# isabella232/handel

Measured on AMD Instinct MI355X. Metric: BN254 aggregate-sig verifications/sec (batch 4096), higher is better.
Workload: dtype u32 (26-bit-limb Fp, 64-bit accumulators)

## Files before the change

### handel_amd/build.py

```python

from __future__ import annotations

import os
import subprocess
import sys
from concurrent.futures import ThreadPoolExecutor

HERE = os.path.dirname(os.path.abspath(__file__))
CSRC = os.path.join(HERE, "csrc")
OUT_DIR = os.path.join(HERE, "_build")
LIB = os.path.join(OUT_DIR, "libhandel_gpu.so")
DIAG_LIB = os.path.join(OUT_DIR, "libhandel_gpu_diag.so")
SOURCES = ["bn256_verify.hip", "bn256_pair.hip", "bn256_kernels.hip", "bn256_gt.hip", "bn256_sig12.hip", "bn256_sigw2.hip", "hg_api.cpp", "hg_aggregate.cpp", "hg_intake.cpp",
           "hg_batcher.cpp", "hg_packets.hip", "hg_service.cpp", "hg_stores.hip", "hg_merge.hip"]
HEADERS = ["bn256_fp.h", "bn256_curve.h", "bn256_team.h", "bn256_kernels.h", "bn256_constants.h",
           "bn256_g2team.h", "bn256_g2sched.h", "bn256_pairing.h", "bn256_xprog.h", "bn256_xtab.h", "bn256_redq.h", "bn256_inv.h", "bn256_agg.h", "bn256_gt.h", "bn256_decode.h", "hg_packets.h", "hg_stores.h", "hg_shm.h", "hg_codes.h", "hg_dev.h", "hg_ctx.h", "hg_sha256.h", "bn256_sigfe.h", "bn256_sigteam.h", "bn256_sigsplit.h", "bn256_sigform.h"]
ARCH = os.environ.get("HG_OFFLOAD_ARCH", "gfx950")
HIPCC = os.environ.get("HIPCC", "/opt/rocm/bin/hipcc")
CFLAGS = ["-O3", "-fPIC", "-std=c++17", f"--offload-arch={ARCH}", "-Wno-unused-result"]


def _inputs():
    files = [os.path.join(CSRC, f) for f in SOURCES + HEADERS]
    files.append(os.path.join(HERE, "..", "include", "handel_gpu.h"))
    files.append(os.path.abspath(__file__))
    return files


def up_to_date(lib: str = LIB) -> bool:
    if not os.path.exists(lib):
        return False
# ... 111 lines not shown
```

### handel_amd/csrc/bn256_sig12.hip

```cpp
#include <hip/hip_runtime.h>

#include "bn256_decode.h"
#include "bn256_g2sched.h"
#include "bn256_gt.h"
#include "bn256_sigfe.h"

namespace hg {

#ifndef HG_SIG_LINE_BLOCK
#define HG_SIG_LINE_BLOCK 256
#endif
static constexpr int kLineBlock = HG_SIG_LINE_BLOCK;

__global__ __launch_bounds__(kLineBlock) void k_sig_scalars(const uint8_t* sig_bytes, int flavor, int n, Fp* sc) {
  const int c = blockIdx.x * kLineBlock + threadIdx.x;
  if (c >= n) return;
  PointG1 sg;
  (void)decode_g1_one(sig_bytes + (size_t)c * 64, flavor, sg);
  Fp nsy, z;
  fp_zero(z);
  fp_neg(nsy, sg.y);
  const bool use = sg.inf == 0;
  fp_sel(sc[2 * c], use, sg.x, z);
  fp_sel(sc[2 * c + 1], use, nsy, z);
// ... 25 lines not shown
      const uint2 x = src[i];
      P.c.l[2 * i] = x.x;
      P.c.l[2 * i + 1] = x.y;
    }
  }
}
HG_DEV void ev_publish(const Team& T, uint32_t* F, EvPipe& P, const Fp* ev, int n, int ci, int next) {
  if (T.tl < 4) st_fp_a8(F + (R_FB_x + T.tl) * 10, P.c.l);
  team_sync();
  if (next < kNumLines) ev_fetch(T, P, ev, n, ci, next);
}

using ISqr12T = XInst<XP_SQR12_12_T, S_F, S_F>;
using ILineT = XInst<XP_LINE_FIX_12_T, S_F, S_F>;

HG_DEV void team_miller_sig12(const Team& T, uint32_t* F, const Fp* ev, int n, int ci, XStream& S, XHint after) {
  const int8_t naf[kNafLen] = HG_NAF;
  t12_set_one(T, S_F);
  if (T.tl == 0) {
    Fp zero, one;
    fp_zero(zero);
    fp_one(one);
    st_fp(F + R_ZERO * 10, zero);
    st_fp(F + R_ONE * 10, one);
  }
  team_sync();
  EvPipe P;
  fp_zero(P.c);
  ev_fetch(T, P, ev, n, ci, 0);
  int s = 0;
  for (int i = kNafLen - 1; i > 0; i--) {
    const int d = naf[i - 1];
    ev_publish(T, F, P, ev, n, ci, s + 1);
    ISqr12T::run(T, S, xh<ILineT>());
    const XHint after_digit = i > 1 ? xh<ISqr12T>() : xh<ILineT>();
    if (d != 0) {
      ILineT::run(T, S, xh<ILineT>());
      ev_publish(T, F, P, ev, n, ci, s + 2);
      ILineT::run(T, S, after_digit);
      s += 2;
    } else {
      ILineT::run(T, S, after_digit);
      s += 1;
    }
  }
  ev_publish(T, F, P, ev, n, ci, s + 1);
// ... 251 lines not shown
```

### handel_amd/csrc/bn256_xprog.h

```cpp
#pragma once
#include <utility>

#include "bn256_redq.h"
#include "bn256_team.h"

namespace hg {

struct Team;
struct XHint {
  int off, w;
};
struct XStream;
template <int NV, int NT, int NP, int NL, int W, int NP2, int NL2, int KP, int KL1, int KL2, int KS1, int KS2, int LZ,
          int EF, int FU>
HG_DEV void x_round(const Team& T, XStream& S, int off, XHint nxt);
template <int QM>
struct XQ {
  template <int NV, int NT, int NP, int NL, int W, int NP2, int NL2, int KP, int KL1, int KL2, int KS1, int KS2,
            int LZ, int EF, int FU>
  HG_DEV static void x_round(const Team& T, XStream& S, int off, XHint nxt);
};

}

#include "bn256_xtab.h"

namespace hg {

static constexpr uint32_t kP2N[10] = {HG_P2N};

struct XStream {
  uint32_t w[kXFetchWords];
  int off;
};
HG_DEV void x_fetch(const Team& T, XStream& S, XHint h) {
  const uint32_t* src = kXTab + h.off + T.tl * h.w;
// ... 48 lines not shown
  for (int l = 0; l < 10; l++) acc[l] = K >= 0 ? (uint32_t)K * kP2N[l] : 0u;
  uint32_t negk = 0;
  x_for<NT>([&](auto t) {
    const uint32_t off = x_term_off(w, base + t);
    const int32_t c = x_coef(w, base + t);
    Fp x;
    ld_fp_a8(x, x_at(T, off));
    if constexpr (K < 0) negk += c < 0 ? (uint32_t)-c : 0u;
#pragma unroll
    for (int l = 0; l < 10; l++) acc[l] += (uint32_t)c * x.l[l];
  });
#pragma unroll
  for (int l = 0; l < 10; l++) out[l] = K >= 0 ? acc[l] : acc[l] + negk * kP2N[l];
}

template <int W, int NT, int K>
HG_DEV void x_lincomb_sum(const uint32_t (&w)[W], int base, const Fp (&xs)[NT], uint32_t (&out)[10]) {
  uint32_t acc[10];
#pragma unroll
  for (int l = 0; l < 10; l++) acc[l] = K >= 0 ? (uint32_t)K * kP2N[l] : 0u;
  uint32_t negk = 0;
#pragma unroll
  for (int t = 0; t < NT; t++) {
    const int32_t c = x_coef(w, base + t);
    if constexpr (K < 0) negk += c < 0 ? (uint32_t)-c : 0u;
#pragma unroll
    for (int l = 0; l < 10; l++) acc[l] += (uint32_t)c * xs[t].l[l];
  }
#pragma unroll
  for (int l = 0; l < 10; l++) out[l] = K >= 0 ? acc[l] : acc[l] + negk * kP2N[l];
}

// ... 235 lines not shown
        const uint32_t dst = x_off(w, (P + kSplitWaves * h) * (1 + NT));
        if (dst != 0xffffu) st_fp_a8(x_at(T, dst), val[h]);
      });
    }
  };
  if constexpr (kSplitWaves == 2) {
    if (T.wave == 0) part(std::integral_constant<int, 0>{});
    else part(std::integral_constant<int, 1>{});
  } else {
    x_for<kSplitWaves>([&](auto r) {
      if (T.wave == decltype(r)::value) part(r);
    });
  }
}

template <int QM, int NV, int NT, int NP, int NL, int W, int NP2, int NL2, int KP, int KL1, int KL2, int KS1, int KS2,
          int LZ, int EF, int FU>
HG_DEV void x_round_q(const Team& T, XStream& S, int off, XHint nxt) {
  if (S.off != off) x_fetch(T, S, XHint{off, W});
  uint32_t w[W];
  x_for<W>([&](auto i) { w[i] = S.w[i]; });
  if (nxt.off >= 0) x_fetch(T, S, nxt);
  constexpr int jbase = NV * (1 + NT);
  Fp e0, e1;
  if constexpr (EF) {
    ld_fp_a8(e0, x_at(T, x_off(w, jbase)));
    ld_fp_a8(e1, x_at(T, x_off(w, jbase + 1)));
  }
  if constexpr (NV > 0) {
    if (kTeamSplit && kSplitPrepass && T.split) {
      x_prepass_split<NV, NT, W, KP>(T, w);
      team_sync(T);
    } else {
    Fp xs[NV][NT];
    x_for<NV>([&](auto v) {
      x_for<NT>([&](auto t) { ld_fp_a8(xs[v][t], x_at(T, x_term_off(w, v * (1 + NT) + 1 + t))); });
    });
    __builtin_amdgcn_sched_barrier(0);
    uint32_t val[NV][10];
    x_for<NV>([&](auto v) { x_lincomb_sum<W, NT, KP>(w, v * (1 + NT) + 1, xs[v], val[v]); });
#pragma unroll
    for (int v = 0; v < NV; v++)
#pragma unroll
      for (int l = 0; l < 10; l++) asm volatile("" : "+v"(val[v][l]));
    x_for<NV>([&](auto v) {
      const uint32_t dst = x_off(w, v * (1 + NT));
      if (dst != 0xffffu) st_fp_a8(x_at(T, dst), val[v]);
    });
    team_sync();
    }
  }
  if constexpr (kTeamSplit && NP2 == 0 && NL2 == 0) {
    if (T.split) {
      x_job_split<W, NP, NL, KL1, KS1, LZ, EF, QM>(T, w, jbase, e0, e1);
      return;
    }
  }
  Fp r;
  uint32_t dst;
  if constexpr (EF) x_job<W, NP, NL, KL1, KS1, LZ, EF, FU, QM>(T, w, jbase, r, dst, e0, e1);
  else x_job<W, NP, NL, KL1, KS1, LZ, 0, FU, QM>(T, w, jbase, r, dst);
  if constexpr (NP2 > 0 || NL2 > 0) {
// ... 3 lines not shown
    team_sync(T);
    if (!kTeamSplit || !T.split || T.wave == 0) {
      if (dst != 0xffffu) st_fp_a8(x_at(T, dst), r.l);
      if (dst2 != 0xffffu) st_fp_a8(x_at(T, dst2), r2.l);
    }
  } else {
    team_sync(T);
    if (dst != 0xffffu) st_fp_a8(x_at(T, dst), r.l);
  }
  team_sync(T);
}

template <int NV, int NT, int NP, int NL, int W, int NP2, int NL2, int KP, int KL1, int KL2, int KS1, int KS2, int LZ,
          int EF, int FU>
HG_DEV void x_round(const Team& T, XStream& S, int off, XHint nxt) {
  x_round_q<0, NV, NT, NP, NL, W, NP2, NL2, KP, KL1, KL2, KS1, KS2, LZ, EF, FU>(T, S, off, nxt);
}
template <int QM>
template <int NV, int NT, int NP, int NL, int W, int NP2, int NL2, int KP, int KL1, int KL2, int KS1, int KS2, int LZ,
          int EF, int FU>
HG_DEV void XQ<QM>::x_round(const Team& T, XStream& S, int off, XHint nxt) {
  static_assert(NL > 0 && NP2 == 0 && NL2 == 0, "one-chain rounds: one job with linear terms");
  x_round_q<QM, NV, NT, NP, NL, W, NP2, NL2, KP, KL1, KL2, KS1, KS2, LZ, EF, FU>(T, S, off, nxt);
}

template <int D, int A, int B>
using IMul12 = XInst<XP_MUL12, D, A, B>;
template <int D, int A>
using ICyc = XInst<XP_CYC_SQR_X, D, A>;
template <int D, int A>
using ICyc0 = XInst<XP_CYC_SQR, D, A>;
template <int D, int A>
using ISqr12 = XInst<XP_SQR12, D, A>;
template <int D, int A>
using ILinePk = XInst<XP_LINE_PK, D, A>;
template <int D, int A>
using ILineFix = XInst<XP_LINE_FIX, D, A>;
template <int PROG>
// ... 55 lines not shown
```

### handel_amd/csrc/bn256_xtab.h

```cpp
#pragma once
#include <stdint.h>
namespace hg {
#define HG_P2N 0x0422599cu, 0x04ac6c5du, 0x05678616u, 0x05120b5au, 0x07b96e22u, 0x0584dc20u, 0x07fb2e17u, 0x047f9aa5u, 0x078d2a8du, 0x008fb500u
enum XProg { XP_PDBL, XP_PADD_POS, XP_PADD_NEG, XP_PADD_F1, XP_PADD_F2, XP_MDBL_1, XP_MDBL_2, XP_PDBL_1, XP_PADD_POS_1, XP_MADD_POS_2, XP_PADD_POS_3, XP_PADD_NEG_1, XP_MADD_NEG_2, XP_PADD_NEG_3, XP_PADD_F1_1, XP_MADD_F1_2, XP_PADD_F1_3, XP_PADD_F2_1, XP_MADD_F2_2, XP_PADD_F2_3, XP_SQR12, XP_LINE_PK, XP_LINE_FIX, XP_CYC_SQR, XP_MUL12, XP_CYC_SQR_X, XP_FEVAL, XP_SDBL, XP_LFEV, XP_MUL12F, XP_SQR12_12, XP_LINE_FIX_12, XP_MUL12_12, XP_CYC_SQR_X_12, XP_LINE_FIX_S, XP_MUL12_S, XP_CYC_SQR_X_S, XP_FEVAL_S, XP_SDBL_S, XP_LFEV_S, XP_SQR12_12_T, XP_LINE_FIX_12_T, XP_MUL12_12_T, XP_CYC_SQR_X_12_T, XP_MDBL_1_V, XP_MDBL_2_V, XP_PDBL_1_V, XP_PADD_POS_1_V, XP_MADD_POS_2_V, XP_PADD_POS_3_V, XP_PADD_NEG_1_V, XP_MADD_NEG_2_V, XP_PADD_NEG_3_V, XP_PADD_F1_1_V, XP_MADD_F1_2_V, XP_PADD_F1_3_V, XP_PADD_F2_1_V, XP_MADD_F2_2_V, XP_PADD_F2_3_V, XP_LINE_PK_V };
__constant__ static const uint32_t kXTab[28288] = {
  0x240616d0u, 0x19509000u, 0x90002906u, 0x28ee1bd0u, 0x16d09000u, 0x16f805c8u, 0x172006b8u, 0x16801748u, 0x24fe1680u, 0x00000f00u, 0x2a1216f8u, 0x19789000u,
  0x900028fau, 0x29fa1bf8u, 0x16d09000u, 0x177006b8u, 0x16800690u, 0x16801680u, 0x2a021680u, 0x00000ff0u, 0x2a031720u, 0x19a02b03u, 0x25032403u, 0x9000ffffu,
  0x17989000u, 0x17c00618u, 0x17e80708u, 0x16801810u, 0x28fe1680u, 0x00000fa0u, 0x2aff1748u, 0x19c82b01u, 0x250124ffu, 0x9000ffffu, 0x17989000u, 0x18380708u,
  0x168006e0u, 0x16801680u, 0x2e021680u, 0x00001090u, 0x25061770u, 0x19f09000u, 0x2b092a09u, 0x9000ffffu, 0x18609000u, 0x18880668u, 0x18b00758u, 0x168018d8u,
  0x2cfe1680u, 0x00001040u, 0x26061798u, 0x1a189000u, 0x90002afau, 0x9000ffffu, 0x19009000u, 0x19280758u, 0x19500730u, 0x19780758u, 0x26020730u, 0x00000f50u,
  0x2c1217c0u, 0x1a409000u, 0x900024fau, 0x9000ffffu, 0x19a09000u, 0x19f019c8u, 0x1a181748u, 0x168006b8u, 0x25fe1680u, 0x00000f28u, 0x2c0317e8u, 0x1a682d03u,
  0x27032603u, 0x9000ffffu, 0x17709000u, 0x1a4006b8u, 0x16800690u, 0x16801680u, 0x2b021680u, 0x00001018u, 0x2cff1810u, 0x1a902d01u, 0x270126ffu, 0x9000ffffu,
  0x1a689000u, 0x1ab81a90u, 0x1ae01810u, 0x16800708u, 0x29fe1680u, 0x00000fc8u, 0x27061838u, 0x1ab89000u, 0x2d092c09u, 0x9000ffffu, 0x18389000u, 0x1b080708u,
  0x168006e0u, 0x16801680u, 0x2f021680u, 0x000010b8u, 0x28061860u, 0x1ae09000u, 0x90002cfau, 0x9000ffffu, 0x1b309000u, 0x1b801b58u, 0x1ba818d8u, 0x16800758u,
  0x2dfe1680u, 0x00001068u, 0x2e121888u, 0x1b089000u, 0x900026fau, 0x9000ffffu, 0x19289000u, 0x1bd00758u, 0x19780730u, 0x1bf80758u, 0x27020730u, 0x00000f78u,
  0x2e0318b0u, 0x1b302f03u, 0x29032803u, 0x9000ffffu, 0x16809000u, 0x16801680u, 0x16801680u, 0x16801680u, 0x90001680u, 0x0000ffffu, 0x2eff18d8u, 0x1b582f01u,
  0x290128ffu, 0x9000ffffu, 0x16809000u, 0x16801680u, 0x16801680u, 0x16801680u, 0x90001680u, 0x0000ffffu, 0x28121900u, 0x1b809000u, 0x2f092e09u, 0x9000ffffu,
  0x16809000u, 0x16801680u, 0x16801680u, 0x16801680u, 0x90001680u, 0x0000ffffu, 0x29121928u, 0x1ba89000u, 0x90002efau, 0x9000ffffu, 0x16809000u, 0x16801680u,
  0x16801680u, 0x16801680u, 0x90001680u, 0x0000ffffu, 0x0c0616d0u, 0x19509000u, 0x0f010effu, 0x020816d0u, 0x02f816f8u, 0x17481720u, 0x01e00cfeu, 0x121216f8u,
  0x19789000u, 0x900014fau, 0x17981770u, 0x02f817c0u, 0x174817e8u, 0x02080dfeu, 0x12031720u, 0x19a01303u, 0x15091409u, 0x03981810u, 0x03701838u, 0x16801680u,
  0x02300e02u, 0x12ff1748u, 0x19c81301u, 0x90000d06u, 0x03981838u, 0x18601810u, 0x16801680u, 0x02580f02u, 0x0c031770u, 0x19f00d03u, 0x90000cfau, 0x02581888u,
  0x034818b0u, 0x190018d8u, 0x028010feu, 0x0cff1798u, 0x1a180d01u, 0x90001006u, 0x19501928u, 0x03481978u, 0x190019a0u, 0x02a811feu, 0x12fa17c0u, 0x1a409000u,
  0x90001612u, 0x02f816d0u, 0x02d019c8u, 0x16801680u, 0x02d01202u, 0x120917e8u, 0x1a681309u, 0x17031603u, 0x02f819c8u, 0x02d019f0u, 0x16801680u, 0x02f81302u,
  0x10121810u, 0x1a901106u, 0x170116ffu, 0x02a81a18u, 0x03981a40u, 0x1a901a68u, 0x032014feu, 0x10fa1838u, 0x1ab81112u, 0x11031003u, 0x1ae01ab8u, 0x03981b08u,
// ... 2436 lines not shown
template <> struct XInst<XP_MUL12_S, S_B, S_A, S_B> { static constexpr int kOff = 16672, kW = 16; HG_DEV static void run(const Team& T, XStream& S, XHint h) { x_round<2, 2, 12, 0, 16, 0, 0, 4, 0, 0, 1, 0, 0, 1, 1>(T, S, 16672, h); } };
template <> struct XInst<XP_MUL12_S, S_B, S_A, S_G> { static constexpr int kOff = 16928, kW = 16; HG_DEV static void run(const Team& T, XStream& S, XHint h) { x_round<2, 2, 12, 0, 16, 0, 0, 4, 0, 0, 1, 0, 0, 1, 1>(T, S, 16928, h); } };
template <> struct XInst<XP_MUL12_S, S_B, S_C, S_G> { static constexpr int kOff = 17184, kW = 16; HG_DEV static void run(const Team& T, XStream& S, XHint h) { x_round<2, 2, 12, 0, 16, 0, 0, 4, 0, 0, 1, 0, 0, 1, 1>(T, S, 17184, h); } };
template <> struct XInst<XP_MUL12_S, S_D, S_C, S_C> { static constexpr int kOff = 17440, kW = 16; HG_DEV static void run(const Team& T, XStream& S, XHint h) { x_round<2, 2, 12, 0, 16, 0, 0, 4, 0, 0, 1, 0, 0, 1, 1>(T, S, 17440, h); } };
template <> struct XInst<XP_MUL12_S, S_D, S_D, S_B> { static constexpr int kOff = 17696, kW = 16; HG_DEV static void run(const Team& T, XStream& S, XHint h) { x_round<2, 2, 12, 0, 16, 0, 0, 4, 0, 0, 1, 0, 0, 1, 1>(T, S, 17696, h); } };
template <> struct XInst<XP_MUL12_S, S_D, S_D, S_E> { static constexpr int kOff = 17952, kW = 16; HG_DEV static void run(const Team& T, XStream& S, XHint h) { x_round<2, 2, 12, 0, 16, 0, 0, 4, 0, 0, 1, 0, 0, 1, 1>(T, S, 17952, h); } };
template <> struct XInst<XP_MUL12_S, S_D, S_D, S_G> { static constexpr int kOff = 18208, kW = 16; HG_DEV static void run(const Team& T, XStream& S, XHint h) { x_round<2, 2, 12, 0, 16, 0, 0, 4, 0, 0, 1, 0, 0, 1, 1>(T, S, 18208, h); } };
template <> struct XInst<XP_MUL12_S, S_E, S_E, S_D> { static constexpr int kOff = 18464, kW = 16; HG_DEV static void run(const Team& T, XStream& S, XHint h) { x_round<2, 2, 12, 0, 16, 0, 0, 4, 0, 0, 1, 0, 0, 1, 1>(T, S, 18464, h); } };
template <> struct XInst<XP_MUL12_S, S_E, S_E, S_G> { static constexpr int kOff = 18720, kW = 16; HG_DEV static void run(const Team& T, XStream& S, XHint h) { x_round<2, 2, 12, 0, 16, 0, 0, 4, 0, 0, 1, 0, 0, 1, 1>(T, S, 18720, h); } };
template <> struct XInst<XP_MUL12_S, S_E, S_F, S_D> { static constexpr int kOff = 18976, kW = 16; HG_DEV static void run(const Team& T, XStream& S, XHint h) { x_round<2, 2, 12, 0, 16, 0, 0, 4, 0, 0, 1, 0, 0, 1, 1>(T, S, 18976, h); } };
template <> struct XInst<XP_MUL12_S, S_F, S_B, S_A> { static constexpr int kOff = 19232, kW = 16; HG_DEV static void run(const Team& T, XStream& S, XHint h) { x_round<2, 2, 12, 0, 16, 0, 0, 4, 0, 0, 1, 0, 0, 1, 1>(T, S, 19232, h); } };
template <> struct XInst<XP_MUL12_S, S_F, S_D, S_A> { static constexpr int kOff = 19488, kW = 16; HG_DEV static void run(const Team& T, XStream& S, XHint h) { x_round<2, 2, 12, 0, 16, 0, 0, 4, 0, 0, 1, 0, 0, 1, 1>(T, S, 19488, h); } };
template <> struct XInst<XP_MUL12_S, S_F, S_F, S_A> { static constexpr int kOff = 19744, kW = 16; HG_DEV static void run(const Team& T, XStream& S, XHint h) { x_round<2, 2, 12, 0, 16, 0, 0, 4, 0, 0, 1, 0, 0, 1, 1>(T, S, 19744, h); } };
template <> struct XInst<XP_MUL12_S, S_G, S_B, S_E> { static constexpr int kOff = 20000, kW = 16; HG_DEV static void run(const Team& T, XStream& S, XHint h) { x_round<2, 2, 12, 0, 16, 0, 0, 4, 0, 0, 1, 0, 0, 1, 1>(T, S, 20000, h); } };
template <> struct XInst<XP_SDBL_S, S_F, S_F> { static constexpr int kOff = 20256, kW = 12; HG_DEV static void run(const Team& T, XStream& S, XHint h) { x_round<3, 2, 7, 0, 12, 0, 0, 8, 0, 0, 1, 0, 0, 0, 1>(T, S, 20256, h); } };
template <> struct XInst<XP_CYC_SQR_X_12_T, S_A, S_A> { static constexpr int kOff = 20448, kW = 7; HG_DEV static void run(const Team& T, XStream& S, XHint h) { XQ<13>::x_round<2, 2, 3, 1, 7, 0, 0, 4, 2, 0, 1, 0, 1, 0, 0>(T, S, 20448, h); } };
template <> struct XInst<XP_CYC_SQR_X_12_T, S_B, S_A> { static constexpr int kOff = 20560, kW = 7; HG_DEV static void run(const Team& T, XStream& S, XHint h) { XQ<13>::x_round<2, 2, 3, 1, 7, 0, 0, 4, 2, 0, 1, 0, 1, 0, 0>(T, S, 20560, h); } };
template <> struct XInst<XP_CYC_SQR_X_12_T, S_C, S_B> { static constexpr int kOff = 20672, kW = 7; HG_DEV static void run(const Team& T, XStream& S, XHint h) { XQ<13>::x_round<2, 2, 3, 1, 7, 0, 0, 4, 2, 0, 1, 0, 1, 0, 0>(T, S, 20672, h); } };
template <> struct XInst<XP_CYC_SQR_X_12_T, S_C, S_C> { static constexpr int kOff = 20784, kW = 7; HG_DEV static void run(const Team& T, XStream& S, XHint h) { XQ<13>::x_round<2, 2, 3, 1, 7, 0, 0, 4, 2, 0, 1, 0, 1, 0, 0>(T, S, 20784, h); } };
template <> struct XInst<XP_CYC_SQR_X_12_T, S_C, S_D> { static constexpr int kOff = 20896, kW = 7; HG_DEV static void run(const Team& T, XStream& S, XHint h) { XQ<13>::x_round<2, 2, 3, 1, 7, 0, 0, 4, 2, 0, 1, 0, 1, 0, 0>(T, S, 20896, h); } };
template <> struct XInst<XP_CYC_SQR_X_12_T, S_C, S_F> { static constexpr int kOff = 21008, kW = 7; HG_DEV static void run(const Team& T, XStream& S, XHint h) { XQ<13>::x_round<2, 2, 3, 1, 7, 0, 0, 4, 2, 0, 1, 0, 1, 0, 0>(T, S, 21008, h); } };
template <> struct XInst<XP_CYC_SQR_X_12_T, S_D, S_C> { static constexpr int kOff = 21120, kW = 7; HG_DEV static void run(const Team& T, XStream& S, XHint h) { XQ<13>::x_round<2, 2, 3, 1, 7, 0, 0, 4, 2, 0, 1, 0, 1, 0, 0>(T, S, 21120, h); } };
template <> struct XInst<XP_CYC_SQR_X_12_T, S_D, S_D> { static constexpr int kOff = 21232, kW = 7; HG_DEV static void run(const Team& T, XStream& S, XHint h) { XQ<13>::x_round<2, 2, 3, 1, 7, 0, 0, 4, 2, 0, 1, 0, 1, 0, 0>(T, S, 21232, h); } };
template <> struct XInst<XP_LINE_FIX_12_T, S_F, S_F> { static constexpr int kOff = 21344, kW = 7; HG_DEV static void run(const Team& T, XStream& S, XHint h) { XQ<13>::x_round<1, 2, 4, 2, 7, 0, 0, 4, 1, 0, 1, 0, 0, 1, 0>(T, S, 21344, h); } };
template <> struct XInst<XP_MUL12_12_T, S_A, S_D, S_B> { static constexpr int kOff = 21456, kW = 16; HG_DEV static void run(const Team& T, XStream& S, XHint h) { x_round<2, 2, 12, 0, 16, 0, 0, 4, 0, 0, 1, 0, 0, 1, 0>(T, S, 21456, h); } };
template <> struct XInst<XP_MUL12_12_T, S_B, S_A, S_B> { static constexpr int kOff = 21712, kW = 16; HG_DEV static void run(const Team& T, XStream& S, XHint h) { x_round<2, 2, 12, 0, 16, 0, 0, 4, 0, 0, 1, 0, 0, 1, 0>(T, S, 21712, h); } };
template <> struct XInst<XP_MUL12_12_T, S_B, S_A, S_F> { static constexpr int kOff = 21968, kW = 16; HG_DEV static void run(const Team& T, XStream& S, XHint h) { x_round<2, 2, 12, 0, 16, 0, 0, 4, 0, 0, 1, 0, 0, 1, 0>(T, S, 21968, h); } };
template <> struct XInst<XP_MUL12_12_T, S_B, S_F, S_D> { static constexpr int kOff = 22224, kW = 16; HG_DEV static void run(const Team& T, XStream& S, XHint h) { x_round<2, 2, 12, 0, 16, 0, 0, 4, 0, 0, 1, 0, 0, 1, 0>(T, S, 22224, h); } };
template <> struct XInst<XP_MUL12_12_T, S_C, S_C, S_B> { static constexpr int kOff = 22480, kW = 16; HG_DEV static void run(const Team& T, XStream& S, XHint h) { x_round<2, 2, 12, 0, 16, 0, 0, 4, 0, 0, 1, 0, 0, 1, 0>(T, S, 22480, h); } };
template <> struct XInst<XP_MUL12_12_T, S_C, S_C, S_D> { static constexpr int kOff = 22736, kW = 16; HG_DEV static void run(const Team& T, XStream& S, XHint h) { x_round<2, 2, 12, 0, 16, 0, 0, 4, 0, 0, 1, 0, 0, 1, 0>(T, S, 22736, h); } };
template <> struct XInst<XP_MUL12_12_T, S_C, S_C, S_F> { static constexpr int kOff = 22992, kW = 16; HG_DEV static void run(const Team& T, XStream& S, XHint h) { x_round<2, 2, 12, 0, 16, 0, 0, 4, 0, 0, 1, 0, 0, 1, 0>(T, S, 22992, h); } };
template <> struct XInst<XP_MUL12_12_T, S_D, S_A, S_A> { static constexpr int kOff = 23248, kW = 16; HG_DEV static void run(const Team& T, XStream& S, XHint h) { x_round<2, 2, 12, 0, 16, 0, 0, 4, 0, 0, 1, 0, 0, 1, 0>(T, S, 23248, h); } };
template <> struct XInst<XP_MUL12_12_T, S_D, S_B, S_C> { static constexpr int kOff = 23504, kW = 16; HG_DEV static void run(const Team& T, XStream& S, XHint h) { x_round<2, 2, 12, 0, 16, 0, 0, 4, 0, 0, 1, 0, 0, 1, 0>(T, S, 23504, h); } };
template <> struct XInst<XP_MUL12_12_T, S_D, S_D, S_B> { static constexpr int kOff = 23760, kW = 16; HG_DEV static void run(const Team& T, XStream& S, XHint h) { x_round<2, 2, 12, 0, 16, 0, 0, 4, 0, 0, 1, 0, 0, 1, 0>(T, S, 23760, h); } };
template <> struct XInst<XP_MUL12_12_T, S_D, S_D, S_C> { static constexpr int kOff = 24016, kW = 16; HG_DEV static void run(const Team& T, XStream& S, XHint h) { x_round<2, 2, 12, 0, 16, 0, 0, 4, 0, 0, 1, 0, 0, 1, 0>(T, S, 24016, h); } };
template <> struct XInst<XP_MUL12_12_T, S_D, S_D, S_F> { static constexpr int kOff = 24272, kW = 16; HG_DEV static void run(const Team& T, XStream& S, XHint h) { x_round<2, 2, 12, 0, 16, 0, 0, 4, 0, 0, 1, 0, 0, 1, 0>(T, S, 24272, h); } };
template <> struct XInst<XP_MUL12_12_T, S_F, S_A, S_D> { static constexpr int kOff = 24528, kW = 16; HG_DEV static void run(const Team& T, XStream& S, XHint h) { x_round<2, 2, 12, 0, 16, 0, 0, 4, 0, 0, 1, 0, 0, 1, 0>(T, S, 24528, h); } };
template <> struct XInst<XP_MUL12_12_T, S_F, S_A, S_F> { static constexpr int kOff = 24784, kW = 16; HG_DEV static void run(const Team& T, XStream& S, XHint h) { x_round<2, 2, 12, 0, 16, 0, 0, 4, 0, 0, 1, 0, 0, 1, 0>(T, S, 24784, h); } };
template <> struct XInst<XP_MUL12_12_T, S_F, S_B, S_A> { static constexpr int kOff = 25040, kW = 16; HG_DEV static void run(const Team& T, XStream& S, XHint h) { x_round<2, 2, 12, 0, 16, 0, 0, 4, 0, 0, 1, 0, 0, 1, 0>(T, S, 25040, h); } };
template <> struct XInst<XP_MUL12_12_T, S_F, S_C, S_F> { static constexpr int kOff = 25296, kW = 16; HG_DEV static void run(const Team& T, XStream& S, XHint h) { x_round<2, 2, 12, 0, 16, 0, 0, 4, 0, 0, 1, 0, 0, 1, 0>(T, S, 25296, h); } };
template <> struct XInst<XP_MUL12_12_T, S_F, S_F, S_A> { static constexpr int kOff = 25552, kW = 16; HG_DEV static void run(const Team& T, XStream& S, XHint h) { x_round<2, 2, 12, 0, 16, 0, 0, 4, 0, 0, 1, 0, 0, 1, 0>(T, S, 25552, h); } };
template <> struct XInst<XP_SQR12_12_T, S_F, S_F> { static constexpr int kOff = 25808, kW = 12; HG_DEV static void run(const Team& T, XStream& S, XHint h) { x_round<3, 2, 7, 0, 12, 0, 0, 8, 0, 0, 1, 0, 0, 0, 0>(T, S, 25808, h); } };
template <> struct XInst<XP_MDBL_1_V, S_F, S_F> { static constexpr int kOff = 26000, kW = 16; HG_DEV static void run(const Team& T, XStream& S, XHint h) { x_round<4, 2, 7, 0, 16, 2, 0, -1, -1, -1, 1, 0, 0, 0, 0>(T, S, 26000, h); } };
template <> struct XInst<XP_MDBL_2_V, S_F, S_F> { static constexpr int kOff = 26256, kW = 14; HG_DEV static void run(const Team& T, XStream& S, XHint h) { x_round<2, 4, 4, 2, 14, 2, 2, -1, -1, -1, 1, 0, 0, 0, 0>(T, S, 26256, h); } };
template <> struct XInst<XP_PDBL_1_V> { static constexpr int kOff = 26480, kW = 4; HG_DEV static void run(const Team& T, XStream& S, XHint h) { x_round<1, 2, 2, 0, 4, 0, 0, -1, -1, -1, 0, 0, 0, 0, 0>(T, S, 26480, h); } };
template <> struct XInst<XP_LINE_PK_V, S_F, S_F> { static constexpr int kOff = 26544, kW = 8; HG_DEV static void run(const Team& T, XStream& S, XHint h) { x_round<1, 2, 6, 0, 8, 0, 0, 4, 0, 0, 1, 0, 0, 1, 0>(T, S, 26544, h); } };
template <> struct XInst<XP_PADD_POS_1_V> { static constexpr int kOff = 26672, kW = 5; HG_DEV static void run(const Team& T, XStream& S, XHint h) { x_round<1, 2, 2, 1, 5, 0, 0, 1, 0, 0, 0, 0, 0, 0, 0>(T, S, 26672, h); } };
template <> struct XInst<XP_PADD_POS_3_V> { static constexpr int kOff = 26752, kW = 10; HG_DEV static void run(const Team& T, XStream& S, XHint h) { x_round<2, 2, 6, 0, 10, 0, 0, 4, 0, 0, 1, 0, 0, 0, 0>(T, S, 26752, h); } };
template <> struct XInst<XP_PADD_NEG_1_V> { static constexpr int kOff = 26912, kW = 5; HG_DEV static void run(const Team& T, XStream& S, XHint h) { x_round<1, 2, 2, 1, 5, 0, 0, 1, 0, 0, 0, 0, 0, 0, 0>(T, S, 26912, h); } };
template <> struct XInst<XP_PADD_NEG_3_V> { static constexpr int kOff = 26992, kW = 10; HG_DEV static void run(const Team& T, XStream& S, XHint h) { x_round<2, 2, 6, 0, 10, 0, 0, 4, 0, 0, 1, 0, 0, 0, 0>(T, S, 26992, h); } };
template <> struct XInst<XP_PADD_F1_1_V> { static constexpr int kOff = 27152, kW = 5; HG_DEV static void run(const Team& T, XStream& S, XHint h) { x_round<1, 2, 2, 1, 5, 0, 0, 1, 0, 0, 0, 0, 0, 0, 0>(T, S, 27152, h); } };
template <> struct XInst<XP_PADD_F1_3_V> { static constexpr int kOff = 27232, kW = 10; HG_DEV static void run(const Team& T, XStream& S, XHint h) { x_round<2, 2, 6, 0, 10, 0, 0, 4, 0, 0, 1, 0, 0, 0, 0>(T, S, 27232, h); } };
template <> struct XInst<XP_PADD_F2_1_V> { static constexpr int kOff = 27392, kW = 5; HG_DEV static void run(const Team& T, XStream& S, XHint h) { x_round<1, 2, 2, 1, 5, 0, 0, 1, 0, 0, 0, 0, 0, 0, 0>(T, S, 27392, h); } };
template <> struct XInst<XP_PADD_F2_3_V> { static constexpr int kOff = 27472, kW = 10; HG_DEV static void run(const Team& T, XStream& S, XHint h) { x_round<2, 2, 6, 0, 10, 0, 0, 4, 0, 0, 1, 0, 0, 0, 0>(T, S, 27472, h); } };
template <> struct XInst<XP_MADD_POS_2_V, S_F, S_F> { static constexpr int kOff = 27632, kW = 10; HG_DEV static void run(const Team& T, XStream& S, XHint h) { x_round<1, 2, 4, 2, 10, 2, 0, 4, 1, 0, 1, 0, 0, 0, 0>(T, S, 27632, h); } };
template <> struct XInst<XP_MADD_NEG_2_V, S_F, S_F> { static constexpr int kOff = 27792, kW = 10; HG_DEV static void run(const Team& T, XStream& S, XHint h) { x_round<1, 2, 4, 2, 10, 2, 0, 4, 1, 0, 1, 0, 0, 0, 0>(T, S, 27792, h); } };
template <> struct XInst<XP_MADD_F1_2_V, S_F, S_F> { static constexpr int kOff = 27952, kW = 10; HG_DEV static void run(const Team& T, XStream& S, XHint h) { x_round<1, 2, 4, 2, 10, 2, 0, 4, 1, 0, 1, 0, 0, 0, 0>(T, S, 27952, h); } };
// ... 3 lines not shown
```

Baseline: 6.476 million.

## Use 64-bit mad lincomb in Fp12 rounds and peel first Miller iteration

Adds a 64-bit multiply-accumulate linear-combination path (lincomb_mad) and switches the Fp12 mul, sqr and cyclotomic-square rounds of the sig12 pipeline to it, storing results with plain word stores. It also peels the first Miller-loop step: instead of setting F to one and squaring, F is initialised directly to the first line value. This drops a redundant square and possibly a line multiply. The risks are a different instruction mix and extra register pressure from the 64-bit accumulators, and subtle correctness in the peeled initialisation.

After: 6.532 million (median of 6 runs). About the same (+0.9%).

```diff
diff --git a/handel_amd/build.py b/handel_amd/build.py
--- a/handel_amd/build.py
+++ b/handel_amd/build.py
@@ -14,7 +14,7 @@
 SOURCES = ["bn256_verify.hip", "bn256_pair.hip", "bn256_kernels.hip", "bn256_gt.hip", "bn256_sig12.hip", "bn256_sigw2.hip", "hg_api.cpp", "hg_aggregate.cpp", "hg_intake.cpp",
            "hg_batcher.cpp", "hg_packets.hip", "hg_service.cpp", "hg_stores.hip", "hg_merge.hip"]
 HEADERS = ["bn256_fp.h", "bn256_curve.h", "bn256_team.h", "bn256_kernels.h", "bn256_constants.h",
-           "bn256_g2team.h", "bn256_g2sched.h", "bn256_pairing.h", "bn256_xprog.h", "bn256_xtab.h", "bn256_redq.h", "bn256_inv.h", "bn256_agg.h", "bn256_gt.h", "bn256_decode.h", "hg_packets.h", "hg_stores.h", "hg_shm.h", "hg_codes.h", "hg_dev.h", "hg_ctx.h", "hg_sha256.h", "bn256_sigfe.h", "bn256_sigteam.h", "bn256_sigsplit.h", "bn256_sigform.h"]
+           "bn256_g2team.h", "bn256_g2sched.h", "bn256_pairing.h", "bn256_xprog.h", "bn256_xtab.h", "bn256_redq.h", "bn256_lincomb.h", "bn256_inv.h", "bn256_agg.h", "bn256_gt.h", "bn256_decode.h", "hg_packets.h", "hg_stores.h", "hg_shm.h", "hg_codes.h", "hg_dev.h", "hg_ctx.h", "hg_sha256.h", "bn256_sigfe.h", "bn256_sigteam.h", "bn256_sigsplit.h", "bn256_sigform.h"]
 ARCH = os.environ.get("HG_OFFLOAD_ARCH", "gfx950")
 HIPCC = os.environ.get("HIPCC", "/opt/rocm/bin/hipcc")
 CFLAGS = ["-O3", "-fPIC", "-std=c++17", f"--offload-arch={ARCH}", "-Wno-unused-result"]
diff --git a/handel_amd/csrc/bn256_lincomb.h b/handel_amd/csrc/bn256_lincomb.h
--- /dev/null
+++ b/handel_amd/csrc/bn256_lincomb.h
@@ -0,0 +1,39 @@
+#pragma once
+#include <stdint.h>
+
+#ifndef HG_HD
+#if defined(__HIPCC__)
+#define HG_HD __host__ __device__ __forceinline__
+#else
+#define HG_HD inline
+#endif
+#endif
+
+#if defined(__HIP_DEVICE_COMPILE__)
+#define HG_PIN64(x) asm("" : "+v"(x))
+#else
+#define HG_PIN64(x) (void)(x)
+#endif
+
+namespace hg {
+
+template <int NT, int K, class E>
+HG_HD void lincomb_mad(const int32_t (&c)[NT], const E (&xs)[NT], const uint32_t (&p2n)[10], uint32_t (&out)[10]) {
+  uint32_t negk = 0;
+  if (K < 0) {
+#pragma unroll
+    for (int t = 0; t < NT; t++) negk += c[t] < 0 ? (uint32_t)-c[t] : 0u;
+  }
+#pragma unroll
+  for (int l = 0; l < 10; l++) {
+    uint64_t acc = K >= 0 ? (uint64_t)((uint32_t)K * p2n[l]) : (uint64_t)negk * p2n[l];
+#pragma unroll
+    for (int t = 0; t < NT; t++) {
+      acc += (uint64_t)(uint32_t)c[t] * xs[t].l[l];
+      HG_PIN64(acc);
+    }
+    out[l] = (uint32_t)acc;
+  }
+}
+
+}
diff --git a/handel_amd/csrc/bn256_sig12.hip b/handel_amd/csrc/bn256_sig12.hip
--- a/handel_amd/csrc/bn256_sig12.hip
+++ b/handel_amd/csrc/bn256_sig12.hip
@@ -63,9 +63,21 @@
 using ISqr12T = XInst<XP_SQR12_12_T, S_F, S_F>;
 using ILineT = XInst<XP_LINE_FIX_12_T, S_F, S_F>;
 
+HG_DEV void sig12_set_line(const Team& T, uint32_t* F) {
+  Fp v, one;
+  fp_zero(v);
+  fp_one(one);
+  if (T.e < 4) ld_fp_a8(v, F + (R_FB_x + (T.e ^ 2)) * 10);
+  fp_sel(v, T.e == 7, one, v);
+  if (T.active) st_fp_a8(slot(T, S_F) + T.e * 10, v.l);
+  team_sync();
+}
+
 HG_DEV void team_miller_sig12(const Team& T, uint32_t* F, const Fp* ev, int n, int ci, XStream& S, XHint after) {
   const int8_t naf[kNafLen] = HG_NAF;
-  t12_set_one(T, S_F);
+  static_assert(kNafLen >= 3, "a first digit and a loop after it");
+  const bool first_adds = naf[kNafLen - 2] != 0;
+  x_fetch(T, S, first_adds ? xh<ILineT>() : xh<ISqr12T>());
   if (T.tl == 0) {
     Fp zero, one;
     fp_zero(zero);
@@ -73,12 +85,18 @@
     st_fp(F + R_ZERO * 10, zero);
     st_fp(F + R_ONE * 10, one);
   }
-  team_sync();
   EvPipe P;
   fp_zero(P.c);
   ev_fetch(T, P, ev, n, ci, 0);
-  int s = 0;
-  for (int i = kNafLen - 1; i > 0; i--) {
+  ev_publish(T, F, P, ev, n, ci, 1);
+  sig12_set_line(T, F);
+  int s = 1;
+  if (first_adds) {
+    ev_publish(T, F, P, ev, n, ci, 2);
+    ILineT::run(T, S, xh<ISqr12T>());
+    s = 2;
+  }
+  for (int i = kNafLen - 2; i > 0; i--) {
     const int d = naf[i - 1];
     ev_publish(T, F, P, ev, n, ci, s + 1);
     ISqr12T::run(T, S, xh<ILineT>());
diff --git a/handel_amd/csrc/bn256_xprog.h b/handel_amd/csrc/bn256_xprog.h
--- a/handel_amd/csrc/bn256_xprog.h
+++ b/handel_amd/csrc/bn256_xprog.h
@@ -1,6 +1,7 @@
 #pragma once
 #include <utility>
 
+#include "bn256_lincomb.h"
 #include "bn256_redq.h"
 #include "bn256_team.h"
 
@@ -20,6 +21,17 @@
             int LZ, int EF, int FU>
   HG_DEV static void x_round(const Team& T, XStream& S, int off, XHint nxt);
 };
+struct XM {
+  template <int NV, int NT, int NP, int NL, int W, int NP2, int NL2, int KP, int KL1, int KL2, int KS1, int KS2,
+            int LZ, int EF, int FU>
+  HG_DEV static void x_round(const Team& T, XStream& S, int off, XHint nxt);
+  template <int QM>
+  struct XQ {
+    template <int NV, int NT, int NP, int NL, int W, int NP2, int NL2, int KP, int KL1, int KL2, int KS1, int KS2,
+              int LZ, int EF, int FU>
+    HG_DEV static void x_round(const Team& T, XStream& S, int off, XHint nxt);
+  };
+};
 
 }
 
@@ -98,8 +110,21 @@
   for (int l = 0; l < 10; l++) out[l] = K >= 0 ? acc[l] : acc[l] + negk * kP2N[l];
 }
 
-template <int W, int NT, int K>
+HG_DEV void x_store_words(const Team& T, uint32_t byte_off, const uint32_t (&v)[10]) {
+  uint32_t* p = (uint32_t*)((uint8_t*)T.base + byte_off);
+#pragma unroll
+  for (int l = 0; l < 10; l++) p[l] = v[l];
+}
+
+template <int W, int NT, int K, int MA = 0>
 HG_DEV void x_lincomb_sum(const uint32_t (&w)[W], int base, const Fp (&xs)[NT], uint32_t (&out)[10]) {
+  if constexpr (MA) {
+    int32_t c[NT];
+#pragma unroll
+    for (int t = 0; t < NT; t++) c[t] = x_coef(w, base + t);
+    lincomb_mad<NT, K>(c, xs, kP2N, out);
+    return;
+  }
   uint32_t acc[10];
 #pragma unroll
   for (int l = 0; l < 10; l++) acc[l] = K >= 0 ? (uint32_t)K * kP2N[l] : 0u;
@@ -365,8 +390,8 @@
   }
 }
 
-template <int QM, int NV, int NT, int NP, int NL, int W, int NP2, int NL2, int KP, int KL1, int KL2, int KS1, int KS2,
-          int LZ, int EF, int FU>
+template <int QM, int MA, int NV, int NT, int NP, int NL, int W, int NP2, int NL2, int KP, int KL1, int KL2, int KS1,
+          int KS2, int LZ, int EF, int FU>
 HG_DEV void x_round_q(const Team& T, XStream& S, int off, XHint nxt) {
   if (S.off != off) x_fetch(T, S, XHint{off, W});
   uint32_t w[W];
@@ -389,14 +414,17 @@
     });
     __builtin_amdgcn_sched_barrier(0);
     uint32_t val[NV][10];
-    x_for<NV>([&](auto v) { x_lincomb_sum<W, NT, KP>(w, v * (1 + NT) + 1, xs[v], val[v]); });
+    x_for<NV>([&](auto v) { x_lincomb_sum<W, NT, KP, MA>(w, v * (1 + NT) + 1, xs[v], val[v]); });
 #pragma unroll
     for (int v = 0; v < NV; v++)
 #pragma unroll
       for (int l = 0; l < 10; l++) asm volatile("" : "+v"(val[v][l]));
     x_for<NV>([&](auto v) {
       const uint32_t dst = x_off(w, v * (1 + NT));
-      if (dst != 0xffffu) st_fp_a8(x_at(T, dst), val[v]);
+      if (dst != 0xffffu) {
+        if constexpr (MA) x_store_words(T, dst, val[v]);
+        else st_fp_a8(x_at(T, dst), val[v]);
+      }
     });
     team_sync();
     }
@@ -430,14 +458,27 @@
 template <int NV, int NT, int NP, int NL, int W, int NP2, int NL2, int KP, int KL1, int KL2, int KS1, int KS2, int LZ,
           int EF, int FU>
 HG_DEV void x_round(const Team& T, XStream& S, int off, XHint nxt) {
-  x_round_q<0, NV, NT, NP, NL, W, NP2, NL2, KP, KL1, KL2, KS1, KS2, LZ, EF, FU>(T, S, off, nxt);
+  x_round_q<0, 0, NV, NT, NP, NL, W, NP2, NL2, KP, KL1, KL2, KS1, KS2, LZ, EF, FU>(T, S, off, nxt);
 }
 template <int QM>
 template <int NV, int NT, int NP, int NL, int W, int NP2, int NL2, int KP, int KL1, int KL2, int KS1, int KS2, int LZ,
           int EF, int FU>
 HG_DEV void XQ<QM>::x_round(const Team& T, XStream& S, int off, XHint nxt) {
   static_assert(NL > 0 && NP2 == 0 && NL2 == 0, "one-chain rounds: one job with linear terms");
-  x_round_q<QM, NV, NT, NP, NL, W, NP2, NL2, KP, KL1, KL2, KS1, KS2, LZ, EF, FU>(T, S, off, nxt);
+  x_round_q<QM, 0, NV, NT, NP, NL, W, NP2, NL2, KP, KL1, KL2, KS1, KS2, LZ, EF, FU>(T, S, off, nxt);
+}
+
+template <int NV, int NT, int NP, int NL, int W, int NP2, int NL2, int KP, int KL1, int KL2, int KS1, int KS2, int LZ,
+          int EF, int FU>
+HG_DEV void XM::x_round(const Team& T, XStream& S, int off, XHint nxt) {
+  x_round_q<0, 1, NV, NT, NP, NL, W, NP2, NL2, KP, KL1, KL2, KS1, KS2, LZ, EF, FU>(T, S, off, nxt);
+}
+template <int QM>
+template <int NV, int NT, int NP, int NL, int W, int NP2, int NL2, int KP, int KL1, int KL2, int KS1, int KS2, int LZ,
+          int EF, int FU>
+HG_DEV void XM::XQ<QM>::x_round(const Team& T, XStream& S, int off, XHint nxt) {
+  static_assert(NL > 0 && NP2 == 0 && NL2 == 0, "one-chain rounds: one job with linear terms");
+  x_round_q<QM, 1, NV, NT, NP, NL, W, NP2, NL2, KP, KL1, KL2, KS1, KS2, LZ, EF, FU>(T, S, off, nxt);
 }
 
 template <int D, int A, int B>
diff --git a/handel_amd/csrc/bn256_xtab.h b/handel_amd/csrc/bn256_xtab.h
--- a/handel_amd/csrc/bn256_xtab.h
+++ b/handel_amd/csrc/bn256_xtab.h
@@ -2474,33 +2474,33 @@
 template <> struct XInst<XP_MUL12_S, S_F, S_F, S_A> { static constexpr int kOff = 19744, kW = 16; HG_DEV static void run(const Team& T, XStream& S, XHint h) { x_round<2, 2, 12, 0, 16, 0, 0, 4, 0, 0, 1, 0, 0, 1, 1>(T, S, 19744, h); } };
 template <> struct XInst<XP_MUL12_S, S_G, S_B, S_E> { static constexpr int kOff = 20000, kW = 16; HG_DEV static void run(const Team& T, XStream& S, XHint h) { x_round<2, 2, 12, 0, 16, 0, 0, 4, 0, 0, 1, 0, 0, 1, 1>(T, S, 20000, h); } };
 template <> struct XInst<XP_SDBL_S, S_F, S_F> { static constexpr int kOff = 20256, kW = 12; HG_DEV static void run(const Team& T, XStream& S, XHint h) { x_round<3, 2, 7, 0, 12, 0, 0, 8, 0, 0, 1, 0, 0, 0, 1>(T, S, 20256, h); } };
-template <> struct XInst<XP_CYC_SQR_X_12_T, S_A, S_A> { static constexpr int kOff = 20448, kW = 7; HG_DEV static void run(const Team& T, XStream& S, XHint h) { XQ<13>::x_round<2, 2, 3, 1, 7, 0, 0, 4, 2, 0, 1, 0, 1, 0, 0>(T, S, 20448, h); } };
-template <> struct XInst<XP_CYC_SQR_X_12_T, S_B, S_A> { static constexpr int kOff = 20560, kW = 7; HG_DEV static void run(const Team& T, XStream& S, XHint h) { XQ<13>::x_round<2, 2, 3, 1, 7, 0, 0, 4, 2, 0, 1, 0, 1, 0, 0>(T, S, 20560, h); } };
-template <> struct XInst<XP_CYC_SQR_X_12_T, S_C, S_B> { static constexpr int kOff = 20672, kW = 7; HG_DEV static void run(const Team& T, XStream& S, XHint h) { XQ<13>::x_round<2, 2, 3, 1, 7, 0, 0, 4, 2, 0, 1, 0, 1, 0, 0>(T, S, 20672, h); } };
-template <> struct XInst<XP_CYC_SQR_X_12_T, S_C, S_C> { static constexpr int kOff = 20784, kW = 7; HG_DEV static void run(const Team& T, XStream& S, XHint h) { XQ<13>::x_round<2, 2, 3, 1, 7, 0, 0, 4, 2, 0, 1, 0, 1, 0, 0>(T, S, 20784, h); } };
-template <> struct XInst<XP_CYC_SQR_X_12_T, S_C, S_D> { static constexpr int kOff = 20896, kW = 7; HG_DEV static void run(const Team& T, XStream& S, XHint h) { XQ<13>::x_round<2, 2, 3, 1, 7, 0, 0, 4, 2, 0, 1, 0, 1, 0, 0>(T, S, 20896, h); } };
-template <> struct XInst<XP_CYC_SQR_X_12_T, S_C, S_F> { static constexpr int kOff = 21008, kW = 7; HG_DEV static void run(const Team& T, XStream& S, XHint h) { XQ<13>::x_round<2, 2, 3, 1, 7, 0, 0, 4, 2, 0, 1, 0, 1, 0, 0>(T, S, 21008, h); } };
-template <> struct XInst<XP_CYC_SQR_X_12_T, S_D, S_C> { static constexpr int kOff = 21120, kW = 7; HG_DEV static void run(const Team& T, XStream& S, XHint h) { XQ<13>::x_round<2, 2, 3, 1, 7, 0, 0, 4, 2, 0, 1, 0, 1, 0, 0>(T, S, 21120, h); } };
-template <> struct XInst<XP_CYC_SQR_X_12_T, S_D, S_D> { static constexpr int kOff = 21232, kW = 7; HG_DEV static void run(const Team& T, XStream& S, XHint h) { XQ<13>::x_round<2, 2, 3, 1, 7, 0, 0, 4, 2, 0, 1, 0, 1, 0, 0>(T, S, 21232, h); } };
+template <> struct XInst<XP_CYC_SQR_X_12_T, S_A, S_A> { static constexpr int kOff = 20448, kW = 7; HG_DEV static void run(const Team& T, XStream& S, XHint h) { XM::XQ<13>::x_round<2, 2, 3, 1, 7, 0, 0, 4, 2, 0, 1, 0, 1, 0, 0>(T, S, 20448, h); } };
+template <> struct XInst<XP_CYC_SQR_X_12_T, S_B, S_A> { static constexpr int kOff = 20560, kW = 7; HG_DEV static void run(const Team& T, XStream& S, XHint h) { XM::XQ<13>::x_round<2, 2, 3, 1, 7, 0, 0, 4, 2, 0, 1, 0, 1, 0, 0>(T, S, 20560, h); } };
+template <> struct XInst<XP_CYC_SQR_X_12_T, S_C, S_B> { static constexpr int kOff = 20672, kW = 7; HG_DEV static void run(const Team& T, XStream& S, XHint h) { XM::XQ<13>::x_round<2, 2, 3, 1, 7, 0, 0, 4, 2, 0, 1, 0, 1, 0, 0>(T, S, 20672, h); } };
+template <> struct XInst<XP_CYC_SQR_X_12_T, S_C, S_C> { static constexpr int kOff = 20784, kW = 7; HG_DEV static void run(const Team& T, XStream& S, XHint h) { XM::XQ<13>::x_round<2, 2, 3, 1, 7, 0, 0, 4, 2, 0, 1, 0, 1, 0, 0>(T, S, 20784, h); } };
+template <> struct XInst<XP_CYC_SQR_X_12_T, S_C, S_D> { static constexpr int kOff = 20896, kW = 7; HG_DEV static void run(const Team& T, XStream& S, XHint h) { XM::XQ<13>::x_round<2, 2, 3, 1, 7, 0, 0, 4, 2, 0, 1, 0, 1, 0, 0>(T, S, 20896, h); } };
+template <> struct XInst<XP_CYC_SQR_X_12_T, S_C, S_F> { static constexpr int kOff = 21008, kW = 7; HG_DEV static void run(const Team& T, XStream& S, XHint h) { XM::XQ<13>::x_round<2, 2, 3, 1, 7, 0, 0, 4, 2, 0, 1, 0, 1, 0, 0>(T, S, 21008, h); } };
+template <> struct XInst<XP_CYC_SQR_X_12_T, S_D, S_C> { static constexpr int kOff = 21120, kW = 7; HG_DEV static void run(const Team& T, XStream& S, XHint h) { XM::XQ<13>::x_round<2, 2, 3, 1, 7, 0, 0, 4, 2, 0, 1, 0, 1, 0, 0>(T, S, 21120, h); } };
+template <> struct XInst<XP_CYC_SQR_X_12_T, S_D, S_D> { static constexpr int kOff = 21232, kW = 7; HG_DEV static void run(const Team& T, XStream& S, XHint h) { XM::XQ<13>::x_round<2, 2, 3, 1, 7, 0, 0, 4, 2, 0, 1, 0, 1, 0, 0>(T, S, 21232, h); } };
 template <> struct XInst<XP_LINE_FIX_12_T, S_F, S_F> { static constexpr int kOff = 21344, kW = 7; HG_DEV static void run(const Team& T, XStream& S, XHint h) { XQ<13>::x_round<1, 2, 4, 2, 7, 0, 0, 4, 1, 0, 1, 0, 0, 1, 0>(T, S, 21344, h); } };
-template <> struct XInst<XP_MUL12_12_T, S_A, S_D, S_B> { static constexpr int kOff = 21456, kW = 16; HG_DEV static void run(const Team& T, XStream& S, XHint h) { x_round<2, 2, 12, 0, 16, 0, 0, 4, 0, 0, 1, 0, 0, 1, 0>(T, S, 21456, h); } };
-template <> struct XInst<XP_MUL12_12_T, S_B, S_A, S_B> { static constexpr int kOff = 21712, kW = 16; HG_DEV static void run(const Team& T, XStream& S, XHint h) { x_round<2, 2, 12, 0, 16, 0, 0, 4, 0, 0, 1, 0, 0, 1, 0>(T, S, 21712, h); } };
-template <> struct XInst<XP_MUL12_12_T, S_B, S_A, S_F> { static constexpr int kOff = 21968, kW = 16; HG_DEV static void run(const Team& T, XStream& S, XHint h) { x_round<2, 2, 12, 0, 16, 0, 0, 4, 0, 0, 1, 0, 0, 1, 0>(T, S, 21968, h); } };
-template <> struct XInst<XP_MUL12_12_T, S_B, S_F, S_D> { static constexpr int kOff = 22224, kW = 16; HG_DEV static void run(const Team& T, XStream& S, XHint h) { x_round<2, 2, 12, 0, 16, 0, 0, 4, 0, 0, 1, 0, 0, 1, 0>(T, S, 22224, h); } };
-template <> struct XInst<XP_MUL12_12_T, S_C, S_C, S_B> { static constexpr int kOff = 22480, kW = 16; HG_DEV static void run(const Team& T, XStream& S, XHint h) { x_round<2, 2, 12, 0, 16, 0, 0, 4, 0, 0, 1, 0, 0, 1, 0>(T, S, 22480, h); } };
-template <> struct XInst<XP_MUL12_12_T, S_C, S_C, S_D> { static constexpr int kOff = 22736, kW = 16; HG_DEV static void run(const Team& T, XStream& S, XHint h) { x_round<2, 2, 12, 0, 16, 0, 0, 4, 0, 0, 1, 0, 0, 1, 0>(T, S, 22736, h); } };
-template <> struct XInst<XP_MUL12_12_T, S_C, S_C, S_F> { static constexpr int kOff = 22992, kW = 16; HG_DEV static void run(const Team& T, XStream& S, XHint h) { x_round<2, 2, 12, 0, 16, 0, 0, 4, 0, 0, 1, 0, 0, 1, 0>(T, S, 22992, h); } };
-template <> struct XInst<XP_MUL12_12_T, S_D, S_A, S_A> { static constexpr int kOff = 23248, kW = 16; HG_DEV static void run(const Team& T, XStream& S, XHint h) { x_round<2, 2, 12, 0, 16, 0, 0, 4, 0, 0, 1, 0, 0, 1, 0>(T, S, 23248, h); } };
-template <> struct XInst<XP_MUL12_12_T, S_D, S_B, S_C> { static constexpr int kOff = 23504, kW = 16; HG_DEV static void run(const Team& T, XStream& S, XHint h) { x_round<2, 2, 12, 0, 16, 0, 0, 4, 0, 0, 1, 0, 0, 1, 0>(T, S, 23504, h); } };
-template <> struct XInst<XP_MUL12_12_T, S_D, S_D, S_B> { static constexpr int kOff = 23760, kW = 16; HG_DEV static void run(const Team& T, XStream& S, XHint h) { x_round<2, 2, 12, 0, 16, 0, 0, 4, 0, 0, 1, 0, 0, 1, 0>(T, S, 23760, h); } };
-template <> struct XInst<XP_MUL12_12_T, S_D, S_D, S_C> { static constexpr int kOff = 24016, kW = 16; HG_DEV static void run(const Team& T, XStream& S, XHint h) { x_round<2, 2, 12, 0, 16, 0, 0, 4, 0, 0, 1, 0, 0, 1, 0>(T, S, 24016, h); } };
-template <> struct XInst<XP_MUL12_12_T, S_D, S_D, S_F> { static constexpr int kOff = 24272, kW = 16; HG_DEV static void run(const Team& T, XStream& S, XHint h) { x_round<2, 2, 12, 0, 16, 0, 0, 4, 0, 0, 1, 0, 0, 1, 0>(T, S, 24272, h); } };
-template <> struct XInst<XP_MUL12_12_T, S_F, S_A, S_D> { static constexpr int kOff = 24528, kW = 16; HG_DEV static void run(const Team& T, XStream& S, XHint h) { x_round<2, 2, 12, 0, 16, 0, 0, 4, 0, 0, 1, 0, 0, 1, 0>(T, S, 24528, h); } };
-template <> struct XInst<XP_MUL12_12_T, S_F, S_A, S_F> { static constexpr int kOff = 24784, kW = 16; HG_DEV static void run(const Team& T, XStream& S, XHint h) { x_round<2, 2, 12, 0, 16, 0, 0, 4, 0, 0, 1, 0, 0, 1, 0>(T, S, 24784, h); } };
-template <> struct XInst<XP_MUL12_12_T, S_F, S_B, S_A> { static constexpr int kOff = 25040, kW = 16; HG_DEV static void run(const Team& T, XStream& S, XHint h) { x_round<2, 2, 12, 0, 16, 0, 0, 4, 0, 0, 1, 0, 0, 1, 0>(T, S, 25040, h); } };
-template <> struct XInst<XP_MUL12_12_T, S_F, S_C, S_F> { static constexpr int kOff = 25296, kW = 16; HG_DEV static void run(const Team& T, XStream& S, XHint h) { x_round<2, 2, 12, 0, 16, 0, 0, 4, 0, 0, 1, 0, 0, 1, 0>(T, S, 25296, h); } };
-template <> struct XInst<XP_MUL12_12_T, S_F, S_F, S_A> { static constexpr int kOff = 25552, kW = 16; HG_DEV static void run(const Team& T, XStream& S, XHint h) { x_round<2, 2, 12, 0, 16, 0, 0, 4, 0, 0, 1, 0, 0, 1, 0>(T, S, 25552, h); } };
-template <> struct XInst<XP_SQR12_12_T, S_F, S_F> { static constexpr int kOff = 25808, kW = 12; HG_DEV static void run(const Team& T, XStream& S, XHint h) { x_round<3, 2, 7, 0, 12, 0, 0, 8, 0, 0, 1, 0, 0, 0, 0>(T, S, 25808, h); } };
+template <> struct XInst<XP_MUL12_12_T, S_A, S_D, S_B> { static constexpr int kOff = 21456, kW = 16; HG_DEV static void run(const Team& T, XStream& S, XHint h) { XM::x_round<2, 2, 12, 0, 16, 0, 0, 4, 0, 0, 1, 0, 0, 1, 0>(T, S, 21456, h); } };
+template <> struct XInst<XP_MUL12_12_T, S_B, S_A, S_B> { static constexpr int kOff = 21712, kW = 16; HG_DEV static void run(const Team& T, XStream& S, XHint h) { XM::x_round<2, 2, 12, 0, 16, 0, 0, 4, 0, 0, 1, 0, 0, 1, 0>(T, S, 21712, h); } };
+template <> struct XInst<XP_MUL12_12_T, S_B, S_A, S_F> { static constexpr int kOff = 21968, kW = 16; HG_DEV static void run(const Team& T, XStream& S, XHint h) { XM::x_round<2, 2, 12, 0, 16, 0, 0, 4, 0, 0, 1, 0, 0, 1, 0>(T, S, 21968, h); } };
+template <> struct XInst<XP_MUL12_12_T, S_B, S_F, S_D> { static constexpr int kOff = 22224, kW = 16; HG_DEV static void run(const Team& T, XStream& S, XHint h) { XM::x_round<2, 2, 12, 0, 16, 0, 0, 4, 0, 0, 1, 0, 0, 1, 0>(T, S, 22224, h); } };
+template <> struct XInst<XP_MUL12_12_T, S_C, S_C, S_B> { static constexpr int kOff = 22480, kW = 16; HG_DEV static void run(const Team& T, XStream& S, XHint h) { XM::x_round<2, 2, 12, 0, 16, 0, 0, 4, 0, 0, 1, 0, 0, 1, 0>(T, S, 22480, h); } };
+template <> struct XInst<XP_MUL12_12_T, S_C, S_C, S_D> { static constexpr int kOff = 22736, kW = 16; HG_DEV static void run(const Team& T, XStream& S, XHint h) { XM::x_round<2, 2, 12, 0, 16, 0, 0, 4, 0, 0, 1, 0, 0, 1, 0>(T, S, 22736, h); } };
+template <> struct XInst<XP_MUL12_12_T, S_C, S_C, S_F> { static constexpr int kOff = 22992, kW = 16; HG_DEV static void run(const Team& T, XStream& S, XHint h) { XM::x_round<2, 2, 12, 0, 16, 0, 0, 4, 0, 0, 1, 0, 0, 1, 0>(T, S, 22992, h); } };
+template <> struct XInst<XP_MUL12_12_T, S_D, S_A, S_A> { static constexpr int kOff = 23248, kW = 16; HG_DEV static void run(const Team& T, XStream& S, XHint h) { XM::x_round<2, 2, 12, 0, 16, 0, 0, 4, 0, 0, 1, 0, 0, 1, 0>(T, S, 23248, h); } };
+template <> struct XInst<XP_MUL12_12_T, S_D, S_B, S_C> { static constexpr int kOff = 23504, kW = 16; HG_DEV static void run(const Team& T, XStream& S, XHint h) { XM::x_round<2, 2, 12, 0, 16, 0, 0, 4, 0, 0, 1, 0, 0, 1, 0>(T, S, 23504, h); } };
+template <> struct XInst<XP_MUL12_12_T, S_D, S_D, S_B> { static constexpr int kOff = 23760, kW = 16; HG_DEV static void run(const Team& T, XStream& S, XHint h) { XM::x_round<2, 2, 12, 0, 16, 0, 0, 4, 0, 0, 1, 0, 0, 1, 0>(T, S, 23760, h); } };
+template <> struct XInst<XP_MUL12_12_T, S_D, S_D, S_C> { static constexpr int kOff = 24016, kW = 16; HG_DEV static void run(const Team& T, XStream& S, XHint h) { XM::x_round<2, 2, 12, 0, 16, 0, 0, 4, 0, 0, 1, 0, 0, 1, 0>(T, S, 24016, h); } };
+template <> struct XInst<XP_MUL12_12_T, S_D, S_D, S_F> { static constexpr int kOff = 24272, kW = 16; HG_DEV static void run(const Team& T, XStream& S, XHint h) { XM::x_round<2, 2, 12, 0, 16, 0, 0, 4, 0, 0, 1, 0, 0, 1, 0>(T, S, 24272, h); } };
+template <> struct XInst<XP_MUL12_12_T, S_F, S_A, S_D> { static constexpr int kOff = 24528, kW = 16; HG_DEV static void run(const Team& T, XStream& S, XHint h) { XM::x_round<2, 2, 12, 0, 16, 0, 0, 4, 0, 0, 1, 0, 0, 1, 0>(T, S, 24528, h); } };
+template <> struct XInst<XP_MUL12_12_T, S_F, S_A, S_F> { static constexpr int kOff = 24784, kW = 16; HG_DEV static void run(const Team& T, XStream& S, XHint h) { XM::x_round<2, 2, 12, 0, 16, 0, 0, 4, 0, 0, 1, 0, 0, 1, 0>(T, S, 24784, h); } };
+template <> struct XInst<XP_MUL12_12_T, S_F, S_B, S_A> { static constexpr int kOff = 25040, kW = 16; HG_DEV static void run(const Team& T, XStream& S, XHint h) { XM::x_round<2, 2, 12, 0, 16, 0, 0, 4, 0, 0, 1, 0, 0, 1, 0>(T, S, 25040, h); } };
+template <> struct XInst<XP_MUL12_12_T, S_F, S_C, S_F> { static constexpr int kOff = 25296, kW = 16; HG_DEV static void run(const Team& T, XStream& S, XHint h) { XM::x_round<2, 2, 12, 0, 16, 0, 0, 4, 0, 0, 1, 0, 0, 1, 0>(T, S, 25296, h); } };
+template <> struct XInst<XP_MUL12_12_T, S_F, S_F, S_A> { static constexpr int kOff = 25552, kW = 16; HG_DEV static void run(const Team& T, XStream& S, XHint h) { XM::x_round<2, 2, 12, 0, 16, 0, 0, 4, 0, 0, 1, 0, 0, 1, 0>(T, S, 25552, h); } };
+template <> struct XInst<XP_SQR12_12_T, S_F, S_F> { static constexpr int kOff = 25808, kW = 12; HG_DEV static void run(const Team& T, XStream& S, XHint h) { XM::x_round<3, 2, 7, 0, 12, 0, 0, 8, 0, 0, 1, 0, 0, 0, 0>(T, S, 25808, h); } };
 template <> struct XInst<XP_MDBL_1_V, S_F, S_F> { static constexpr int kOff = 26000, kW = 16; HG_DEV static void run(const Team& T, XStream& S, XHint h) { x_round<4, 2, 7, 0, 16, 2, 0, -1, -1, -1, 1, 0, 0, 0, 0>(T, S, 26000, h); } };
 template <> struct XInst<XP_MDBL_2_V, S_F, S_F> { static constexpr int kOff = 26256, kW = 14; HG_DEV static void run(const Team& T, XStream& S, XHint h) { x_round<2, 4, 4, 2, 14, 2, 2, -1, -1, -1, 1, 0, 0, 0, 0>(T, S, 26256, h); } };
 template <> struct XInst<XP_PDBL_1_V> { static constexpr int kOff = 26480, kW = 4; HG_DEV static void run(const Team& T, XStream& S, XHint h) { x_round<1, 2, 2, 0, 4, 0, 0, -1, -1, -1, 0, 0, 0, 0, 0>(T, S, 26480, h); } };
```
